# klausondrag/FOSVOS

Measured on AMD Instinct MI355X. Metric: online fine-tune frames/sec (854x480), higher is better.
Workload: dtype bf16; 1 GPU; OSVOS_VGG train_online one-shot fine-tune: 1x3x480x854 frame per step, fwd + class-balanced BCE + bwd, fused SGD step every 5 steps (BASELINE.json configs[1]); batch=1, avg_grad_every_n=5, activations=bf16 NHWC, fp32 accumulate, fp32 master weights, parallelism=single GPU

## Files before the change

### fosvos_amd/csrc/conv_igemm.hip

```cpp
#include <stdlib.h>

#include "common.hpp"

using namespace fosvos;

namespace {

constexpr unsigned kReluAfterAdd = 0x100u;
constexpr unsigned kSubsample2 = 0x200u;
constexpr unsigned kNoSplitK = 0x400u;

struct ConvArgs {
    const uint16_t *x;
    const uint16_t *w;
    const float *bias;
    const uint16_t *relu_src;
    const uint8_t *relu_bits;
    const uint16_t *addend;
    void *y;
    uint16_t *y_pool;
    const uint16_t *unpool_g;
    int N, H, W, Cin, Cout, Co_pad;
    int tiles_x, tiles_y;
    unsigned flags;
    int swizzle;
    int k_splits;
    int chunks_per_split;
    float *partial;
    unsigned m_ncb, m_nt, m_tx, m_ty;
    int n_t;
#ifdef FOSVOS_STAMP
    unsigned long long *stamps;
#endif
};

#ifdef FOSVOS_STAMP
unsigned long long *g_stamps = nullptr;
#define FOSVOS_STAMP_AT(i)                                                                               \
    if (a.stamps && threadIdx.x == 0)                                                                    \
        a.stamps[((((int64_t)blockIdx.z * gridDim.y + blockIdx.y) * gridDim.x + blockIdx.x) << 4) + (i)] = \
            __builtin_amdgcn_s_memtime();
#define FOSVOS_STAMP_RT(i)                                                                               \
    if (a.stamps && threadIdx.x == 0)                                                                    \
        a.stamps[((((int64_t)blockIdx.z * gridDim.y + blockIdx.y) * gridDim.x + blockIdx.x) << 4) + (i)] = \
            __builtin_amdgcn_s_memrealtime();
#else
#define FOSVOS_STAMP_AT(i)
#define FOSVOS_STAMP_RT(i)
#endif

__device__ __forceinline__ unsigned fast_div(unsigned n, unsigned d, unsigned m) { return m ? __umulhi(n, m) : n / d; }
unsigned recip_mul(int64_t n_max, int64_t d) {
    return (d >= 2 && n_max * d < (int64_t(1) << 32)) ? (unsigned)((int64_t(1) << 32) / d + 1) : 0u;
}

template <int TH_, int TW_, int BN_, int WM_, int WN_>
struct Tile {
    static constexpr int TH = TH_, TW = TW_, BN = BN_, WM = WM_, WN = WN_;
    static constexpr int BM = TH * TW;
    static constexpr int HALO_W = TW + 2, HALO_H = TH + 2;
    static constexpr int NPIX = HALO_W * HALO_H;
    static constexpr int NPIX8 = (NPIX + 7) / 8 * 8;
    static constexpr int NPIX_PAD = (NPIX + 15) / 16 * 16;
    static constexpr int WAVE_M = BM / WM, WAVE_N = BN / WN;
    static constexpr int MF = WAVE_M / 16, NF = WAVE_N / 16;
    static constexpr int A_SLOTS = 4 * NPIX_PAD;
    static constexpr int B_SLOTS = 36 * BN;
    static constexpr int NT = 64 * WM * WN;
    static constexpr int A_IT = (NPIX8 * 4 + NT - 1) / NT;
    static constexpr int B_IT = (B_SLOTS + NT - 1) / NT;
    static constexpr int OUT_LD = BN + 8;
    static constexpr int LDS_MAIN = (A_SLOTS + B_SLOTS) * 16;
    static constexpr int LDS_OUT = BM * OUT_LD * 2;
    static constexpr int LDS_BYTES = LDS_MAIN > LDS_OUT ? LDS_MAIN : LDS_OUT;
#ifndef FOSVOS_MID_WPE
#define FOSVOS_MID_WPE 3
#endif
    static constexpr int WPE = (BM >= 256 || BN < 64) ? 2 : FOSVOS_MID_WPE;
    static_assert(WM * WN == 4 || WM * WN == 8, "4 or 8 waves per workgroup");
    static_assert(TW % 16 == 0 && WAVE_M % 16 == 0 && WAVE_N % 16 == 0, "fragment alignment");
    static_assert(BM % WM == 0 && BN % WN == 0, "wave split");
};

template <int MF, int NF>
struct TapPlan {
    static constexpr int rows_b = MF / 2 > 0 ? MF / 2 : 1;
    static constexpr int per_row = (NF + rows_b - 1) / rows_b;
    static constexpr int nb(int i) {
        const int left = NF - i * per_row;
        return left <= 0 ? 0 : (left < per_row ? left : per_row);
    }
};
template <int MF, int NF, int I, bool NEXT, int V>
__device__ __forceinline__ void sched_row() {
    if constexpr (I < MF) {
        __builtin_amdgcn_sched_group_barrier(0x008, NF, 0);
        if constexpr (NEXT) __builtin_amdgcn_sched_group_barrier(0x100, 1 + TapPlan<MF, NF>::nb(I), 0);
        constexpr int rows_v = V < MF ? V : MF;
        constexpr int nv = I < MF - rows_v ? 0 : (I == MF - 1 ? V - (rows_v - 1) : 1);
        if constexpr (nv > 0) __builtin_amdgcn_sched_group_barrier(0x020, nv, 0);
    }
}
template <int MF, int NF, bool NEXT, int V>
__device__ __forceinline__ void sched_tap() {
    static_assert(MF <= 8, "sched_tap rows");
    sched_row<MF, NF, 0, NEXT, V>(); sched_row<MF, NF, 1, NEXT, V>(); sched_row<MF, NF, 2, NEXT, V>();
    sched_row<MF, NF, 3, NEXT, V>(); sched_row<MF, NF, 4, NEXT, V>(); sched_row<MF, NF, 5, NEXT, V>();
    sched_row<MF, NF, 6, NEXT, V>(); sched_row<MF, NF, 7, NEXT, V>();
}

template <class T, bool OUT_F32, bool UNPOOL = false>
__global__ __launch_bounds__(T::NT) __attribute__((amdgpu_waves_per_eu(2, T::WPE))) void k_conv3x3_igemm(const ConvArgs a) {
    extern __shared__ __attribute__((aligned(16))) uint4 smem[];
    uint4 *sA = smem;
    uint4 *sB = smem + T::A_SLOTS;
#ifdef FOSVOS_IGEMM_PRIO
    __builtin_amdgcn_s_setprio(FOSVOS_IGEMM_PRIO);
#endif

    const int tid = threadIdx.x, lane = tid & 63;
    const int wave = __builtin_amdgcn_readfirstlane(tid >> 6);
    const int wm = wave / T::WN, wn = wave % T::WN;
    int t = blockIdx.x;
    int cb = blockIdx.y;
    if (a.swizzle) {
        const int n_wg = gridDim.x, n_cb = a.Cout / T::BN, n_t = a.n_t;
        const int q8 = n_wg >> 3, r8 = n_wg & 7, xcd = t & 7;
        const int swz = (xcd < r8 ? xcd * (q8 + 1) : r8 * (q8 + 1) + (xcd - r8) * q8) + (t >> 3);
        if (a.swizzle == 1) { t = fast_div(swz, n_cb, a.m_ncb); cb = swz - t * n_cb; }
        else { cb = fast_div(swz, n_t, a.m_nt); t = swz - cb * n_t; }
    }
    const int t_row = fast_div(t, a.tiles_x, a.m_tx);
    const int tx_i = t - t_row * a.tiles_x;
    const int n = fast_div(t_row, a.tiles_y, a.m_ty);
    const int ty_i = t_row - n * a.tiles_y;
    const int y0 = ty_i * T::TH, x0 = tx_i * T::TW;
    const int n0 = cb * T::BN;
    const int H = a.H, W = a.W, Cin = a.Cin;
    const int n_chunks = Cin >> 5;
    const uint16_t *xn = a.x + (int64_t)n * H * W * Cin;

    int a_goff[T::A_IT];
    int a_slot[T::A_IT];
#pragma unroll
    for (int it = 0; it < T::A_IT; ++it) {
        const int idx = it * T::NT + tid;
        const int oct = idx >> 5, within = idx & 31;
        const int kg = within >> 3;
        const int P = oct * 8 + (within & 7);
        a_slot[it] = -1;
        a_goff[it] = -1;
        if (P < T::NPIX) {
            const int hy = P / T::HALO_W, hx = P - hy * T::HALO_W;
            const int gy = y0 + hy - 1, gx = x0 + hx - 1;
            a_slot[it] = kg * T::NPIX_PAD + P;
            if (gy >= 0 && gy < H && gx >= 0 && gx < W) a_goff[it] = ((gy * W + gx) * Cin + kg * 8) * 2;
        }
    }

    f32x4 acc[T::MF][T::NF];
#pragma unroll
    for (int i = 0; i < T::MF; ++i)
#pragma unroll
        for (int j = 0; j < T::NF; ++j) acc[i][j] = f32x4{0.f, 0.f, 0.f, 0.f};

    int a_base[T::MF];
#pragma unroll
    for (int i = 0; i < T::MF; ++i) {
        const int pb = wm * T::WAVE_M + i * 16;
        const int ty = pb / T::TW, tx = pb % T::TW;
        a_base[i] = (lane >> 4) * T::NPIX_PAD + ty * T::HALO_W + tx + (lane & 15);
    }
    const int b_base = (lane >> 4) * T::BN + wn * T::WAVE_N + (lane & 15);

    const int c_begin = a.k_splits > 1 ? blockIdx.z * a.chunks_per_split : 0;
    const int c_end = a.k_splits > 1 ? min(c_begin + a.chunks_per_split, n_chunks) : n_chunks;

    static_assert(T::A_IT <= 6 && T::B_IT <= 9, "prefetch register file");
    uint4 pa0, pa1, pa2, pa3, pa4, pa5, pb0, pb1, pb2, pb3, pb4, pb5, pb6, pb7, pb8;
    [[maybe_unused]] uint4 pa6, pa7, pa8;
    pa0 = pa1 = pa2 = pa3 = pa4 = pa5 = pb0 = pb1 = pb2 = pb3 = pb4 = pb5 = pb6 = pb7 = pb8 = make_uint4(0, 0, 0, 0);
    const int x_bytes = H * W * Cin * 2, w_bytes = (n_chunks * 36 * a.Co_pad - n0) * 16;
    auto x_rsrc = __builtin_amdgcn_make_buffer_rsrc(const_cast<uint16_t *>(xn), 0, x_bytes, 0x00020000);
    auto w_rsrc = __builtin_amdgcn_make_buffer_rsrc(const_cast<uint16_t *>(a.w) + (int64_t)n0 * 8, 0, w_bytes,
                                                    0x00020000);
    static_assert(T::NT % T::BN == 0, "weight staging assumes BN divides the workgroup size");
    const int b_voff = ((tid / T::BN) * a.Co_pad + tid % T::BN) * 16;
    const int b_row_bytes = a.Co_pad * 16;
#define FOSVOS_LD_A(i)                                                                                  \
    if constexpr (i < T::A_IT)                                                                          \
        pa##i = __builtin_bit_cast(uint4, __builtin_amdgcn_raw_buffer_load_b128(x_rsrc, a_goff[i], cc_ * 64, 0));
#define FOSVOS_LD_B(i)                                                                                  \
    if constexpr (i < T::B_IT)                                                                          \
        pb##i = __builtin_bit_cast(uint4, __builtin_amdgcn_raw_buffer_load_b128(                        \
            w_rsrc, b_voff, (cc_ * 36 + i * (T::NT / T::BN)) * b_row_bytes, 0));
#define FOSVOS_LOAD_CHUNK(cc_expr)                                                                      \
    {                                                                                                   \
        const int cc_ = (cc_expr);                                                                      \
        FOSVOS_LD_A(0) FOSVOS_LD_A(1) FOSVOS_LD_A(2) FOSVOS_LD_A(3) FOSVOS_LD_A(4) FOSVOS_LD_A(5)       \
        FOSVOS_LD_B(0) FOSVOS_LD_B(1) FOSVOS_LD_B(2) FOSVOS_LD_B(3) FOSVOS_LD_B(4) FOSVOS_LD_B(5)       \
        FOSVOS_LD_B(6) FOSVOS_LD_B(7) FOSVOS_LD_B(8)                                                    \
    }
#define FOSVOS_ST_A(i)                                                                                  \
    if constexpr (i < T::A_IT) {                                                                        \
        if (a_slot[i] >= 0) sA[a_slot[i]] = pa##i;                                                      \
    }
#define FOSVOS_ST_B(i)                                                                                  \
    if constexpr (i < T::B_IT) {                                                                        \
        if (i * T::NT + tid < T::B_SLOTS) sB[i * T::NT + tid] = pb##i;                                  \
    }
#define FOSVOS_STORE_CHUNK()                                                                            \
    {                                                                                                   \
        FOSVOS_ST_A(0) FOSVOS_ST_A(1) FOSVOS_ST_A(2) FOSVOS_ST_A(3) FOSVOS_ST_A(4) FOSVOS_ST_A(5)       \
        FOSVOS_ST_B(0) FOSVOS_ST_B(1) FOSVOS_ST_B(2) FOSVOS_ST_B(3) FOSVOS_ST_B(4) FOSVOS_ST_B(5)       \
        FOSVOS_ST_B(6) FOSVOS_ST_B(7) FOSVOS_ST_B(8)                                                    \
    }

#define FOSVOS_RD_A(tap_, i_) \
    af[i_] = __builtin_bit_cast(bf16x8, sA[a_base[i_] + ((tap_) / 3) * T::HALO_W + (tap_) % 3]);
#define FOSVOS_RD_B(tap_, buf_, j_) \
    bfr[buf_][j_] = __builtin_bit_cast(bf16x8, sB[b_base + (tap_) * 4 * T::BN + (j_) * 16]);
#define FOSVOS_ROW(tap_, i_)                                                                            \
    if constexpr ((i_) < T::MF) {                                                                       \
        _Pragma("unroll") for (int j = 0; j < T::NF; ++j) acc[i_][j] =                                  \
            __builtin_amdgcn_mfma_f32_16x16x32_bf16(bfr[(tap_) & 1][j], af[i_], acc[i_][j], 0, 0, 0);   \
        if constexpr ((tap_) < 8) {                                                                     \
            FOSVOS_RD_A((tap_) + 1, i_)                                                                 \
            _Pragma("unroll") for (int j = 0; j < TP::nb(i_); ++j)                                      \
                FOSVOS_RD_B((tap_) + 1, ((tap_) + 1) & 1, (i_) * TP::per_row + j)                       \
        }                                                                                               \
    }
#define FOSVOS_TAP(tap_)                                                                                \
    {                                                                                                   \
        FOSVOS_ROW(tap_, 0) FOSVOS_ROW(tap_, 1) FOSVOS_ROW(tap_, 2) FOSVOS_ROW(tap_, 3)                 \
        FOSVOS_ROW(tap_, 4) FOSVOS_ROW(tap_, 5) FOSVOS_ROW(tap_, 6) FOSVOS_ROW(tap_, 7)                 \
        {                                                                                               \
            const int cc_ = cc + 1;                                                                     \
            FOSVOS_LD_B(tap_)                                                                           \
            FOSVOS_LD_A(tap_)                                                                           \
        }                                                                                               \
        sched_tap<T::MF, T::NF, ((tap_) < 8), 1 + ((tap_) < T::A_IT ? 1 : 0)>();                        \
    }

    FOSVOS_STAMP_RT(11)
    FOSVOS_STAMP_AT(0)
    if (c_begin < c_end) FOSVOS_LOAD_CHUNK(c_begin)
    FOSVOS_STAMP_AT(1)
    using TP = TapPlan<T::MF, T::NF>;
    static_assert(T::MF <= 8, "row macros cover up to 8 pixel fragments per wave");
    bf16x8 af[T::MF], bfr[2][T::NF];
    for (int cc = c_begin; cc < c_end; ++cc) {
        if (cc > c_begin) __syncthreads();
        if (cc == c_end - 1) { FOSVOS_STAMP_AT(6) }
        FOSVOS_STORE_CHUNK()
        if (cc == c_begin) { FOSVOS_STAMP_AT(2) }
        if (cc == c_end - 1) { FOSVOS_STAMP_AT(7) }
        __syncthreads();
        if (cc == c_begin) { FOSVOS_STAMP_AT(3) }
#pragma unroll
        for (int i = 0; i < T::MF; ++i) FOSVOS_RD_A(0, i)
#pragma unroll
        for (int j = 0; j < T::NF; ++j) FOSVOS_RD_B(0, 0, j)
        __builtin_amdgcn_sched_group_barrier(0x100, T::MF + T::NF, 0);
        if (cc + 1 == c_end) {
            x_rsrc = __builtin_amdgcn_make_buffer_rsrc(const_cast<uint16_t *>(xn), 0, 0, 0x00020000);
            w_rsrc = __builtin_amdgcn_make_buffer_rsrc(const_cast<uint16_t *>(a.w) + (int64_t)n0 * 8, 0, 0, 0x00020000);
        }
        FOSVOS_TAP(0) FOSVOS_TAP(1) FOSVOS_TAP(2) FOSVOS_TAP(3) FOSVOS_TAP(4) FOSVOS_TAP(5) FOSVOS_TAP(6)
        FOSVOS_TAP(7) FOSVOS_TAP(8)
        if (cc == c_begin) { FOSVOS_STAMP_AT(5) }
    }
    FOSVOS_STAMP_AT(8)

    const int q = lane >> 4, cl = lane & 15;
    if (a.k_splits > 1) {
        float *po = a.partial + (int64_t)blockIdx.z * a.N * H * W * a.Cout;
#pragma unroll
        for (int i = 0; i < T::MF; ++i) {
            const int pix = wm * T::WAVE_M + i * 16 + cl;
            const int gy = y0 + pix / T::TW, gx = x0 + pix % T::TW;
            if (gy < H && gx < W) {
                float *row = po + (((int64_t)n * H + gy) * W + gx) * a.Cout + n0 + wn * T::WAVE_N + q * 4;
#pragma unroll
                for (int j = 0; j < T::NF; ++j)
                    *reinterpret_cast<float4 *>(row + j * 16) =
                        make_float4(acc[i][j][0], acc[i][j][1], acc[i][j][2], acc[i][j][3]);
            }
        }
        return;
    }
    if (OUT_F32) {
        float *yo = reinterpret_cast<float *>(a.y);
#pragma unroll
        for (int j = 0; j < T::NF; ++j) {
            const int co = n0 + wn * T::WAVE_N + j * 16 + q * 4;
            float4 b = make_float4(0.f, 0.f, 0.f, 0.f);
            if (a.bias) b = *reinterpret_cast<const float4 *>(a.bias + co);
#pragma unroll
            for (int i = 0; i < T::MF; ++i) {
                const int pix = wm * T::WAVE_M + i * 16 + cl;
                const int gy = y0 + pix / T::TW, gx = x0 + pix % T::TW;
                if (gy < H && gx < W) {
                    float4 v = make_float4(acc[i][j][0] + b.x, acc[i][j][1] + b.y, acc[i][j][2] + b.z,
                                           acc[i][j][3] + b.w);
                    if (a.flags & FOSVOS_CONV_RELU)
                        v = make_float4(relu_f(v.x), relu_f(v.y), relu_f(v.z), relu_f(v.w));
                    *reinterpret_cast<float4 *>(yo + (((int64_t)n * H + gy) * W + gx) * a.Cout + co) = v;
                }
            }
        }
        return;
    }
    constexpr int VEC_PER_PIX = T::BN / 8;
    constexpr int OUT_N = T::BM * VEC_PER_PIX;
    constexpr int OUT_IT = (OUT_N + T::NT - 1) / T::NT;
    constexpr int PIX_STEP = T::NT / VEC_PER_PIX;
    static_assert(T::NT % VEC_PER_PIX == 0 && PIX_STEP % T::TW == 0, "a thread's output vectors must share a column");
    constexpr int ROW_STEP = PIX_STEP / T::TW;
    const int o_cg = tid % VEC_PER_PIX, o_pix = tid / VEC_PER_PIX;
    const int o_ly = o_pix / T::TW, o_gx = x0 + o_pix % T::TW;
    const int img_bytes = H * W * a.Cout * 2;
    uint16_t *yo = reinterpret_cast<uint16_t *>(a.y);
    int voff[OUT_IT];
#pragma unroll
    for (int it = 0; it < OUT_IT; ++it) {
        const int gy = y0 + o_ly + it * ROW_STEP;
        const bool ok = it * T::NT + tid < OUT_N && gy < H && o_gx < W;
        voff[it] = ok ? ((gy * W + o_gx) * a.Cout + n0 + o_cg * 8) * 2 : -1;
    }
    const bool masked = (a.relu_src || a.relu_bits || a.addend) && !(a.flags & kSubsample2);
    uint4 mk[OUT_IT], ad[OUT_IT];
#pragma unroll
    for (int it = 0; it < OUT_IT; ++it) mk[it] = ad[it] = make_uint4(0, 0, 0, 0);
    if constexpr (UNPOOL) {
        const int OH = (H + 1) >> 1, OW = (W + 1) >> 1;
        auto m_rsrc = __builtin_amdgcn_make_buffer_rsrc(const_cast<uint16_t *>(a.relu_src + (int64_t)n * H * W * a.Cout), 0,
                                                        img_bytes, 0x00020000);
        auto g_rsrc = __builtin_amdgcn_make_buffer_rsrc(const_cast<uint16_t *>(a.unpool_g + (int64_t)n * OH * OW * a.Cout), 0,
                                                        OH * OW * a.Cout * 2, 0x00020000);
#pragma unroll
        for (int it = 0; it < OUT_IT; ++it)
            mk[it] = __builtin_bit_cast(uint4, __builtin_amdgcn_raw_buffer_load_b128(m_rsrc, voff[it], 0, 0));
#pragma unroll
        for (int it = 0; it < OUT_IT; ++it) {
            const int gy = y0 + o_ly + it * ROW_STEP;
            const int goff = voff[it] < 0 ? -1 : (((gy >> 1) * OW + (o_gx >> 1)) * a.Cout + n0 + o_cg * 8) * 2;
            ad[it] = __builtin_bit_cast(uint4, __builtin_amdgcn_raw_buffer_load_b128(g_rsrc, goff, 0, 0));
        }
    } else if (masked && a.relu_bits) {
        auto b_rsrc = __builtin_amdgcn_make_buffer_rsrc(const_cast<uint8_t *>(a.relu_bits + (int64_t)n * H * W * (a.Cout >> 3)), 0,
                                                        img_bytes >> 4, 0x00020000);
#pragma unroll
        for (int it = 0; it < OUT_IT; ++it) {
            const unsigned b = __builtin_amdgcn_raw_buffer_load_b8(b_rsrc, voff[it] < 0 ? -1 : voff[it] >> 4, 0, 0);
            mk[it] = make_uint4((b & 1u) | ((b & 2u) << 15), ((b >> 2) & 1u) | ((b & 8u) << 13), ((b >> 4) & 1u) | ((b & 32u) << 11),
                                ((b >> 6) & 1u) | ((b & 128u) << 9));
        }
        if (a.addend) {
            auto ad_rsrc = __builtin_amdgcn_make_buffer_rsrc(const_cast<uint16_t *>(a.addend + (int64_t)n * H * W * a.Cout), 0,
                                                             img_bytes, 0x00020000);
#pragma unroll
            for (int it = 0; it < OUT_IT; ++it)
                ad[it] = __builtin_bit_cast(uint4, __builtin_amdgcn_raw_buffer_load_b128(ad_rsrc, voff[it], 0, 0));
        }
    } else if (masked) {
        auto m_rsrc = __builtin_amdgcn_make_buffer_rsrc(
            const_cast<uint16_t *>(a.relu_src ? a.relu_src + (int64_t)n * H * W * a.Cout : yo), 0,
            a.relu_src ? img_bytes : 0, 0x00020000);
        auto ad_rsrc = __builtin_amdgcn_make_buffer_rsrc(
            const_cast<uint16_t *>(a.addend ? a.addend + (int64_t)n * H * W * a.Cout : yo), 0,
            a.addend ? img_bytes : 0, 0x00020000);
#pragma unroll
        for (int it = 0; it < OUT_IT; ++it)
            mk[it] = __builtin_bit_cast(uint4, __builtin_amdgcn_raw_buffer_load_b128(m_rsrc, voff[it], 0, 0));
#pragma unroll
        for (int it = 0; it < OUT_IT; ++it)
            ad[it] = __builtin_bit_cast(uint4, __builtin_amdgcn_raw_buffer_load_b128(ad_rsrc, voff[it], 0, 0));
    }
    float4 bias_r[T::NF];
#pragma unroll
    for (int j = 0; j < T::NF; ++j)
        bias_r[j] = a.bias ? *reinterpret_cast<const float4 *>(a.bias + n0 + wn * T::WAVE_N + j * 16 + q * 4)
                           : make_float4(0.f, 0.f, 0.f, 0.f);
    __syncthreads();
    uint16_t *sO = reinterpret_cast<uint16_t *>(smem);
#pragma unroll
    for (int j = 0; j < T::NF; ++j) {
        const int col = wn * T::WAVE_N + j * 16 + q * 4;
        const float4 b = bias_r[j];
#pragma unroll
        for (int i = 0; i < T::MF; ++i) {
            const int pix = wm * T::WAVE_M + i * 16 + cl;
            float v0 = acc[i][j][0] + b.x, v1 = acc[i][j][1] + b.y, v2 = acc[i][j][2] + b.z, v3 = acc[i][j][3] + b.w;
            if (a.flags & FOSVOS_CONV_RELU) {
                v0 = relu_f(v0); v1 = relu_f(v1); v2 = relu_f(v2); v3 = relu_f(v3);
            }
            *reinterpret_cast<uint2 *>(sO + pix * T::OUT_LD + col) = make_uint2(pack2bf(v0, v1), pack2bf(v2, v3));
        }
    }
    if constexpr (UNPOOL) {
        uint16_t *sX = sO + T::BM * T::OUT_LD;
#pragma unroll
        for (int it = 0; it < OUT_IT; ++it)
            if (it * T::NT + tid < OUT_N)
                *reinterpret_cast<uint4 *>(sX + (o_pix + it * PIX_STEP) * T::OUT_LD + o_cg * 8) = mk[it];
    }
    __syncthreads();
    FOSVOS_STAMP_AT(9)
    const uint16_t *s_vec = sO + o_pix * T::OUT_LD + o_cg * 8;
    auto y_rsrc = __builtin_amdgcn_make_buffer_rsrc(yo + (int64_t)n * H * W * a.Cout, 0, img_bytes, 0x00020000);
    if constexpr (UNPOOL) {
        static_assert((T::TW & (T::TW - 1)) == 0 && T::TH % 2 == 0, "window partners are pix ^ 1 and pix ^ TW");
        const uint16_t *sX = sO + T::BM * T::OUT_LD;
        const fosvos_i16x2 one2 = {1, 1}, zero2 = {0, 0};
        const fosvos_i16x2 late_x = (o_pix & 1) ? zero2 : one2;
#pragma unroll
        for (int it = 0; it < OUT_IT; ++it) {
            const int pix = o_pix + it * PIX_STEP;
            if (it * T::NT + tid >= OUT_N) continue;
            const fosvos_i16x2 late_y = (pix & T::TW) ? zero2 : one2;
            const uint4 cv = keep_where_pos_bf16x8(*reinterpret_cast<const uint4 *>(s_vec + it * PIX_STEP * T::OUT_LD), mk[it]);
            const uint4 x1 = *reinterpret_cast<const uint4 *>(sX + (pix ^ 1) * T::OUT_LD + o_cg * 8);
            const uint4 x2 = *reinterpret_cast<const uint4 *>(sX + (pix ^ T::TW) * T::OUT_LD + o_cg * 8);
            const uint4 x3 = *reinterpret_cast<const uint4 *>(sX + (pix ^ T::TW ^ 1) * T::OUT_LD + o_cg * 8);
            auto win = [&](unsigned own_, unsigned p1, unsigned p2, unsigned p3) {
                const fosvos_i16x2 own = __builtin_bit_cast(fosvos_i16x2, own_);
                const fosvos_i16x2 s = (zero2 - own) & (__builtin_bit_cast(fosvos_i16x2, p1) - own - late_x) &
                                       (__builtin_bit_cast(fosvos_i16x2, p2) - own - late_y) &
                                       (__builtin_bit_cast(fosvos_i16x2, p3) - own - late_y);
                return __builtin_bit_cast(unsigned, s >> 15);
            };
            const uint4 routed = make_uint4(ad[it].x & win(mk[it].x, x1.x, x2.x, x3.x), ad[it].y & win(mk[it].y, x1.y, x2.y, x3.y),
                                            ad[it].z & win(mk[it].z, x1.z, x2.z, x3.z), ad[it].w & win(mk[it].w, x1.w, x2.w, x3.w));
            float f[8], r[8];
            unpack8(cv, f);
            unpack8(routed, r);
#pragma unroll
            for (int e = 0; e < 8; ++e) f[e] += r[e];
            __builtin_amdgcn_raw_buffer_store_b128(__builtin_bit_cast(u32x4, pack8(f)), y_rsrc, voff[it], 0, 0);
        }
    } else if (!(a.flags & kSubsample2)) {
        if (masked) {
#pragma unroll
            for (int it = 0; it < OUT_IT; ++it) {
                uint4 v = *reinterpret_cast<const uint4 *>(s_vec + it * PIX_STEP * T::OUT_LD);
                if (a.relu_src || a.relu_bits) v = keep_where_pos_bf16x8(v, mk[it]);
                if (a.addend || (a.flags & kReluAfterAdd)) {
                    float f[8];
                    unpack8(v, f);
                    if (a.addend) {
                        float av[8];
                        unpack8(ad[it], av);
#pragma unroll
                        for (int e = 0; e < 8; ++e) f[e] += av[e];
                    }
                    if (a.flags & kReluAfterAdd) {
#pragma unroll
                        for (int e = 0; e < 8; ++e) f[e] = relu_f(f[e]);
                    }
                    v = pack8(f);
                }
                __builtin_amdgcn_raw_buffer_store_b128(__builtin_bit_cast(u32x4, v), y_rsrc, voff[it], 0, 0);
            }
        } else {
#pragma unroll
            for (int it = 0; it < OUT_IT; ++it)
                __builtin_amdgcn_raw_buffer_store_b128(
                    __builtin_bit_cast(u32x4, *reinterpret_cast<const uint4 *>(s_vec + it * PIX_STEP * T::OUT_LD)), y_rsrc,
                    voff[it], 0, 0);
        }
    } else {
#pragma unroll
        for (int it = 0; it < OUT_IT; ++it) {
            const int gy = y0 + o_ly + it * ROW_STEP;
            if (it * T::NT + tid >= OUT_N || gy >= H || o_gx >= W || ((gy | o_gx) & 1)) continue;
            const int64_t off =
                (((int64_t)n * ((H + 1) >> 1) + (gy >> 1)) * ((W + 1) >> 1) + (o_gx >> 1)) * a.Cout + n0 + o_cg * 8;
            *reinterpret_cast<uint4 *>(yo + off) = *reinterpret_cast<const uint4 *>(s_vec + it * PIX_STEP * T::OUT_LD);
        }
    }
    if (a.y_pool) {
        static_assert(T::TH % 2 == 0 && T::TW % 2 == 0, "pooling windows must not straddle tiles");
        constexpr int PW = T::TW / 2, PN = (T::TH / 2) * PW;
        const int OH = (H + 1) >> 1, OW = (W + 1) >> 1;
        auto p_rsrc = __builtin_amdgcn_make_buffer_rsrc(a.y_pool + (int64_t)n * OH * OW * a.Cout, 0, OH * OW * a.Cout * 2,
                                                        0x00020000);
        for (int idx = tid; idx < PN * VEC_PER_PIX; idx += T::NT) {
            const int pp = idx / VEC_PER_PIX, cg = idx % VEC_PER_PIX;
            const int py = pp / PW, px = pp % PW;
            const int oy = (y0 >> 1) + py, ox = (x0 >> 1) + px;
            if (oy >= OH || ox >= OW) continue;
            const int poff = ((oy * OW + ox) * a.Cout + n0 + cg * 8) * 2;
            if (a.flags & FOSVOS_CONV_RELU) {
                uint4 mx = make_uint4(0, 0, 0, 0);
#pragma unroll
                for (int t = 0; t < 4; ++t) {
                    const int ly = 2 * py + (t >> 1), lx = 2 * px + (t & 1);
                    if (y0 + ly < H && x0 + lx < W)
                        mx = max_nonneg_bf16x8(mx, *reinterpret_cast<const uint4 *>(sO + (ly * T::TW + lx) * T::OUT_LD + cg * 8));
                }
                __builtin_amdgcn_raw_buffer_store_b128(__builtin_bit_cast(u32x4, mx), p_rsrc, poff, 0, 0);
                continue;
            }
            float m[8];
#pragma unroll
            for (int j = 0; j < 8; ++j) m[j] = -INFINITY;
#pragma unroll
            for (int t = 0; t < 4; ++t) {
                const int ly = 2 * py + (t >> 1), lx = 2 * px + (t & 1);
                if (y0 + ly < H && x0 + lx < W) {
                    float f[8];
                    unpack8(*reinterpret_cast<const uint4 *>(sO + (ly * T::TW + lx) * T::OUT_LD + cg * 8), f);
#pragma unroll
                    for (int j = 0; j < 8; ++j) m[j] = f[j] > m[j] ? f[j] : m[j];
                }
            }
            __builtin_amdgcn_raw_buffer_store_b128(__builtin_bit_cast(u32x4, pack8(m)), p_rsrc, poff, 0, 0);
        }
    }
    FOSVOS_STAMP_AT(10)
    FOSVOS_STAMP_RT(12)
}

__global__ __launch_bounds__(256) void k_splitk_epilogue(const ConvArgs a, int64_t total8) {
    const int groups = a.Cout >> 3;
    const int64_t plane = (int64_t)a.N * a.H * a.W * a.Cout;
    for (int64_t i = blockIdx.x * 256LL + threadIdx.x; i < total8; i += (int64_t)gridDim.x * 256) {
        const int g = (int)(i % groups);
        int64_t off = i * 8;
        if (a.flags & kSubsample2) {
            const int Ho = (a.H + 1) >> 1, Wo = (a.W + 1) >> 1;
            int64_t pq = i / groups;
            const int ox = (int)(pq % Wo);
            pq /= Wo;
            const int oy = (int)(pq % Ho), n = (int)(pq / Ho);
            off = (((int64_t)n * a.H + 2 * oy) * a.W + 2 * ox) * a.Cout + g * 8;
        }
        float f[8];
#pragma unroll
        for (int e = 0; e < 8; ++e) f[e] = 0.f;
        for (int z0 = 0; z0 < a.k_splits; z0 += 4) {
            float4 v0[4], v1[4];
#pragma unroll
            for (int j = 0; j < 4; ++j) {
                const int z = min(z0 + j, a.k_splits - 1);
                v0[j] = *reinterpret_cast<const float4 *>(a.partial + z * plane + off);
                v1[j] = *reinterpret_cast<const float4 *>(a.partial + z * plane + off + 4);
            }
#pragma unroll
            for (int j = 0; j < 4; ++j) {
                if (z0 + j < a.k_splits) {
                    f[0] += v0[j].x; f[1] += v0[j].y; f[2] += v0[j].z; f[3] += v0[j].w;
                    f[4] += v1[j].x; f[5] += v1[j].y; f[6] += v1[j].z; f[7] += v1[j].w;
                }
            }
        }
        if (a.bias) {
#pragma unroll
            for (int e = 0; e < 8; ++e) f[e] += a.bias[g * 8 + e];
        }
        if (a.flags & FOSVOS_CONV_RELU) {
#pragma unroll
            for (int e = 0; e < 8; ++e) f[e] = relu_f(f[e]);
        }
        if (a.flags & FOSVOS_CONV_OUT_F32) {
            float *yo = reinterpret_cast<float *>(a.y) + off;
            *reinterpret_cast<float4 *>(yo) = make_float4(f[0], f[1], f[2], f[3]);
            *reinterpret_cast<float4 *>(yo + 4) = make_float4(f[4], f[5], f[6], f[7]);
            continue;
        }
        if (a.relu_src || a.relu_bits || a.addend) {
            uint4 v = pack8(f);
            unpack8(v, f);
// ... 373 lines not shown
```

Before: 1235 frames/s.

## Overlap LDS chunk store with last-tap MFMAs and spread prefetch loads across taps

Restructures the implicit-GEMM conv main loop so the last tap's MFMAs interleave with the LDS stores of the next chunk, with an explicit waitcnt plus barrier before them. The loop is peeled so the final chunk runs without prefetch. Global prefetch loads are now spread evenly over the first six taps instead of one per tap. Invalid store slots are redirected to spare LDS slots, which removes the per-store branches. The aim is to hide LDS store and barrier latency behind compute, at the cost of an extra barrier per chunk and more register pressure.

Result: no change. 1249 frames/s, median of 6 (+1.1%).

```diff
diff --git a/fosvos_amd/csrc/conv_igemm.hip b/fosvos_amd/csrc/conv_igemm.hip
--- a/fosvos_amd/csrc/conv_igemm.hip
+++ b/fosvos_amd/csrc/conv_igemm.hip
@@ -90,6 +90,13 @@
         const int left = NF - i * per_row;
         return left <= 0 ? 0 : (left < per_row ? left : per_row);
     }
+    static constexpr int kLoadTaps = 6;
+    static constexpr int load_tap(int l, int n_loads) { return l * kLoadTaps / n_loads; }
+    static constexpr int loads_in_tap(int tap, int n_loads) {
+        int n = 0;
+        for (int l = 0; l < n_loads; ++l) n += load_tap(l, n_loads) == tap ? 1 : 0;
+        return n;
+    }
 };
 template <int MF, int NF, int I, bool NEXT, int V>
 __device__ __forceinline__ void sched_row() {
@@ -107,6 +114,16 @@
     sched_row<MF, NF, 0, NEXT, V>(); sched_row<MF, NF, 1, NEXT, V>(); sched_row<MF, NF, 2, NEXT, V>();
     sched_row<MF, NF, 3, NEXT, V>(); sched_row<MF, NF, 4, NEXT, V>(); sched_row<MF, NF, 5, NEXT, V>();
     sched_row<MF, NF, 6, NEXT, V>(); sched_row<MF, NF, 7, NEXT, V>();
+}
+
+template <int NM, int NS, int K = 0>
+__device__ __forceinline__ void sched_store() {
+    if constexpr (K < NM) {
+        __builtin_amdgcn_sched_group_barrier(0x008, 1, 0);
+        constexpr int nw = ((K + 1) * NS + NM - 1) / NM - (K * NS + NM - 1) / NM;
+        if constexpr (nw > 0) __builtin_amdgcn_sched_group_barrier(0x200, nw, 0);
+        sched_store<NM, NS, K + 1>();
+    }
 }
 
 template <class T, bool OUT_F32, bool UNPOOL = false>
@@ -176,45 +193,49 @@
     const int c_begin = a.k_splits > 1 ? blockIdx.z * a.chunks_per_split : 0;
     const int c_end = a.k_splits > 1 ? min(c_begin + a.chunks_per_split, n_chunks) : n_chunks;
 
+    constexpr int NL = T::A_IT + T::B_IT;
     static_assert(T::A_IT <= 6 && T::B_IT <= 9, "prefetch register file");
-    uint4 pa0, pa1, pa2, pa3, pa4, pa5, pb0, pb1, pb2, pb3, pb4, pb5, pb6, pb7, pb8;
-    [[maybe_unused]] uint4 pa6, pa7, pa8;
-    pa0 = pa1 = pa2 = pa3 = pa4 = pa5 = pb0 = pb1 = pb2 = pb3 = pb4 = pb5 = pb6 = pb7 = pb8 = make_uint4(0, 0, 0, 0);
+    [[maybe_unused]] uint4 p0, p1, p2, p3, p4, p5, p6, p7, p8, p9, p10, p11, p12, p13, p14;
+    p0 = p1 = p2 = p3 = p4 = p5 = p6 = p7 = p8 = p9 = p10 = p11 = p12 = p13 = p14 = make_uint4(0, 0, 0, 0);
     const int x_bytes = H * W * Cin * 2, w_bytes = (n_chunks * 36 * a.Co_pad - n0) * 16;
-    auto x_rsrc = __builtin_amdgcn_make_buffer_rsrc(const_cast<uint16_t *>(xn), 0, x_bytes, 0x00020000);
-    auto w_rsrc = __builtin_amdgcn_make_buffer_rsrc(const_cast<uint16_t *>(a.w) + (int64_t)n0 * 8, 0, w_bytes,
-                                                    0x00020000);
+    const auto x_rsrc = __builtin_amdgcn_make_buffer_rsrc(const_cast<uint16_t *>(xn), 0, x_bytes, 0x00020000);
+    const auto w_rsrc = __builtin_amdgcn_make_buffer_rsrc(const_cast<uint16_t *>(a.w) + (int64_t)n0 * 8, 0, w_bytes,
+                                                          0x00020000);
     static_assert(T::NT % T::BN == 0, "weight staging assumes BN divides the workgroup size");
     const int b_voff = ((tid / T::BN) * a.Co_pad + tid % T::BN) * 16;
     const int b_row_bytes = a.Co_pad * 16;
-#define FOSVOS_LD_A(i)                                                                                  \
-    if constexpr (i < T::A_IT)                                                                          \
-        pa##i = __builtin_bit_cast(uint4, __builtin_amdgcn_raw_buffer_load_b128(x_rsrc, a_goff[i], cc_ * 64, 0));
-#define FOSVOS_LD_B(i)                                                                                  \
-    if constexpr (i < T::B_IT)                                                                          \
-        pb##i = __builtin_bit_cast(uint4, __builtin_amdgcn_raw_buffer_load_b128(                        \
-            w_rsrc, b_voff, (cc_ * 36 + i * (T::NT / T::BN)) * b_row_bytes, 0));
+    constexpr int SPARE = T::NPIX_PAD - T::NPIX;
+    static_assert(SPARE > 0, "the input image needs spare slots");
+    const int spare_slot = T::NPIX + tid % SPARE;
+#pragma unroll
+    for (int it = 0; it < T::A_IT; ++it)
+        if (a_slot[it] < 0) a_slot[it] = spare_slot;
+    constexpr int B_TAIL = T::B_IT - 1;
+    const int b_tail_slot = B_TAIL * T::NT + tid < T::B_SLOTS ? T::A_SLOTS + B_TAIL * T::NT + tid : spare_slot;
+#define FOSVOS_LD_(l)                                                                                   \
+    if constexpr ((l) < T::A_IT)                                                                        \
+        p##l = __builtin_bit_cast(uint4, __builtin_amdgcn_raw_buffer_load_b128(x_rsrc, a_goff[(l)], cc_ * 64, 0)); \
+    else if constexpr ((l) < NL)                                                                        \
+        p##l = __builtin_bit_cast(uint4, __builtin_amdgcn_raw_buffer_load_b128(                         \
+            w_rsrc, b_voff, (cc_ * 36 + ((l) - T::A_IT) * (T::NT / T::BN)) * b_row_bytes, 0));
+#define FOSVOS_LD_ALL(M_, x_)                                                                           \
+    M_(0, x_) M_(1, x_) M_(2, x_) M_(3, x_) M_(4, x_) M_(5, x_) M_(6, x_) M_(7, x_) M_(8, x_) M_(9, x_)   \
+    M_(10, x_) M_(11, x_) M_(12, x_) M_(13, x_) M_(14, x_)
+#define FOSVOS_LD_ANY(l, x_) FOSVOS_LD_(l)
+#define FOSVOS_LD_IN_TAP(l, tap_) \
+    if constexpr ((l) < NL && TP::load_tap((l), NL) == (tap_)) { FOSVOS_LD_(l) }
 #define FOSVOS_LOAD_CHUNK(cc_expr)                                                                      \
     {                                                                                                   \
         const int cc_ = (cc_expr);                                                                      \
-        FOSVOS_LD_A(0) FOSVOS_LD_A(1) FOSVOS_LD_A(2) FOSVOS_LD_A(3) FOSVOS_LD_A(4) FOSVOS_LD_A(5)       \
-        FOSVOS_LD_B(0) FOSVOS_LD_B(1) FOSVOS_LD_B(2) FOSVOS_LD_B(3) FOSVOS_LD_B(4) FOSVOS_LD_B(5)       \
-        FOSVOS_LD_B(6) FOSVOS_LD_B(7) FOSVOS_LD_B(8)                                                    \
-    }
-#define FOSVOS_ST_A(i)                                                                                  \
-    if constexpr (i < T::A_IT) {                                                                        \
-        if (a_slot[i] >= 0) sA[a_slot[i]] = pa##i;                                                      \
-    }
-#define FOSVOS_ST_B(i)                                                                                  \
-    if constexpr (i < T::B_IT) {                                                                        \
-        if (i * T::NT + tid < T::B_SLOTS) sB[i * T::NT + tid] = pb##i;                                  \
-    }
-#define FOSVOS_STORE_CHUNK()                                                                            \
-    {                                                                                                   \
-        FOSVOS_ST_A(0) FOSVOS_ST_A(1) FOSVOS_ST_A(2) FOSVOS_ST_A(3) FOSVOS_ST_A(4) FOSVOS_ST_A(5)       \
-        FOSVOS_ST_B(0) FOSVOS_ST_B(1) FOSVOS_ST_B(2) FOSVOS_ST_B(3) FOSVOS_ST_B(4) FOSVOS_ST_B(5)       \
-        FOSVOS_ST_B(6) FOSVOS_ST_B(7) FOSVOS_ST_B(8)                                                    \
-    }
+        FOSVOS_LD_ALL(FOSVOS_LD_ANY, 0)                                                                 \
+    }
+#define FOSVOS_ST(l, x_)                                                                                \
+    if constexpr ((l) < T::A_IT) sA[a_slot[(l)]] = p##l;                                                \
+    else if constexpr ((l) < NL) {                                                                      \
+        if constexpr (((l) - T::A_IT + 1) * T::NT <= T::B_SLOTS) sB[((l) - T::A_IT) * T::NT + tid] = p##l; \
+        else smem[b_tail_slot] = p##l;                                                                  \
+    }
+#define FOSVOS_STORE_CHUNK() { FOSVOS_LD_ALL(FOSVOS_ST, 0) }
 
 #define FOSVOS_RD_A(tap_, i_) \
     af[i_] = __builtin_bit_cast(bf16x8, sA[a_base[i_] + ((tap_) / 3) * T::HALO_W + (tap_) % 3]);
@@ -230,45 +251,61 @@
                 FOSVOS_RD_B((tap_) + 1, ((tap_) + 1) & 1, (i_) * TP::per_row + j)                       \
         }                                                                                               \
     }
+#define FOSVOS_ROWS(tap_)                                                                               \
+    FOSVOS_ROW(tap_, 0) FOSVOS_ROW(tap_, 1) FOSVOS_ROW(tap_, 2) FOSVOS_ROW(tap_, 3)                     \
+    FOSVOS_ROW(tap_, 4) FOSVOS_ROW(tap_, 5) FOSVOS_ROW(tap_, 6) FOSVOS_ROW(tap_, 7)
 #define FOSVOS_TAP(tap_)                                                                                \
     {                                                                                                   \
-        FOSVOS_ROW(tap_, 0) FOSVOS_ROW(tap_, 1) FOSVOS_ROW(tap_, 2) FOSVOS_ROW(tap_, 3)                 \
-        FOSVOS_ROW(tap_, 4) FOSVOS_ROW(tap_, 5) FOSVOS_ROW(tap_, 6) FOSVOS_ROW(tap_, 7)                 \
+        FOSVOS_ROWS(tap_)                                                                               \
         {                                                                                               \
             const int cc_ = cc + 1;                                                                     \
-            FOSVOS_LD_B(tap_)                                                                           \
-            FOSVOS_LD_A(tap_)                                                                           \
+            FOSVOS_LD_ALL(FOSVOS_LD_IN_TAP, tap_)                                                       \
         }                                                                                               \
-        sched_tap<T::MF, T::NF, ((tap_) < 8), 1 + ((tap_) < T::A_IT ? 1 : 0)>();                        \
-    }
-
-    FOSVOS_STAMP_RT(11)
-    FOSVOS_STAMP_AT(0)
-    if (c_begin < c_end) FOSVOS_LOAD_CHUNK(c_begin)
-    FOSVOS_STAMP_AT(1)
+        sched_tap<T::MF, T::NF, true, TP::loads_in_tap((tap_), NL)>();                                  \
+    }
+#define FOSVOS_TAP_LAST(tap_)                                                                           \
+    {                                                                                                   \
+        FOSVOS_ROWS(tap_)                                                                               \
+        sched_tap<T::MF, T::NF, ((tap_) < 8), 0>();                                                     \
+    }
+#define FOSVOS_FIRST_READS()                                                                            \
+    {                                                                                                   \
+        _Pragma("unroll") for (int i = 0; i < T::MF; ++i) FOSVOS_RD_A(0, i)                             \
+        _Pragma("unroll") for (int j = 0; j < T::NF; ++j) FOSVOS_RD_B(0, 0, j)                          \
+        __builtin_amdgcn_sched_group_barrier(0x100, T::MF + T::NF, 0);                                  \
+    }
+
     using TP = TapPlan<T::MF, T::NF>;
     static_assert(T::MF <= 8, "row macros cover up to 8 pixel fragments per wave");
     bf16x8 af[T::MF], bfr[2][T::NF];
-    for (int cc = c_begin; cc < c_end; ++cc) {
-        if (cc > c_begin) __syncthreads();
-        if (cc == c_end - 1) { FOSVOS_STAMP_AT(6) }
+    FOSVOS_STAMP_RT(11)
+    FOSVOS_STAMP_AT(0)
+    if (c_begin < c_end) {
+        FOSVOS_LOAD_CHUNK(c_begin)
+        FOSVOS_STAMP_AT(1)
         FOSVOS_STORE_CHUNK()
-        if (cc == c_begin) { FOSVOS_STAMP_AT(2) }
-        if (cc == c_end - 1) { FOSVOS_STAMP_AT(7) }
+        FOSVOS_STAMP_AT(2)
         __syncthreads();
-        if (cc == c_begin) { FOSVOS_STAMP_AT(3) }
-#pragma unroll
-        for (int i = 0; i < T::MF; ++i) FOSVOS_RD_A(0, i)
-#pragma unroll
-        for (int j = 0; j < T::NF; ++j) FOSVOS_RD_B(0, 0, j)
-        __builtin_amdgcn_sched_group_barrier(0x100, T::MF + T::NF, 0);
-        if (cc + 1 == c_end) {
-            x_rsrc = __builtin_amdgcn_make_buffer_rsrc(const_cast<uint16_t *>(xn), 0, 0, 0x00020000);
-            w_rsrc = __builtin_amdgcn_make_buffer_rsrc(const_cast<uint16_t *>(a.w) + (int64_t)n0 * 8, 0, 0, 0x00020000);
-        }
-        FOSVOS_TAP(0) FOSVOS_TAP(1) FOSVOS_TAP(2) FOSVOS_TAP(3) FOSVOS_TAP(4) FOSVOS_TAP(5) FOSVOS_TAP(6)
-        FOSVOS_TAP(7) FOSVOS_TAP(8)
-        if (cc == c_begin) { FOSVOS_STAMP_AT(5) }
+        FOSVOS_STAMP_AT(3)
+        FOSVOS_FIRST_READS()
+        for (int cc = c_begin; cc + 1 < c_end; ++cc) {
+            FOSVOS_TAP(0) FOSVOS_TAP(1) FOSVOS_TAP(2) FOSVOS_TAP(3) FOSVOS_TAP(4) FOSVOS_TAP(5) FOSVOS_TAP(6)
+            FOSVOS_TAP(7)
+            if (cc == c_begin) { FOSVOS_STAMP_AT(5) }
+            if (cc + 2 == c_end) { FOSVOS_STAMP_AT(6) }
+            __builtin_amdgcn_s_waitcnt(0xc07f);
+            __syncthreads();
+            if (cc + 2 == c_end) { FOSVOS_STAMP_AT(13) }
+            FOSVOS_ROWS(8)
+            FOSVOS_STORE_CHUNK()
+            sched_store<T::MF * T::NF, NL>();
+            if (cc + 2 == c_end) { FOSVOS_STAMP_AT(7) }
+            __syncthreads();
+            FOSVOS_FIRST_READS()
+            if (cc + 2 == c_end) { FOSVOS_STAMP_AT(14) }
+        }
+        FOSVOS_TAP_LAST(0) FOSVOS_TAP_LAST(1) FOSVOS_TAP_LAST(2) FOSVOS_TAP_LAST(3) FOSVOS_TAP_LAST(4)
+        FOSVOS_TAP_LAST(5) FOSVOS_TAP_LAST(6) FOSVOS_TAP_LAST(7) FOSVOS_TAP_LAST(8)
     }
     FOSVOS_STAMP_AT(8)
 
```
